# jim-berend/semanticlens

Hardware: AMD Instinct MI355X
Metric: images/sec concept-db build (higher is better)
Workload: dtype f32 (encoder GEMMs split-bf16x3, fp32 accumulate)

## Files before the change

include/semanticlens_amd.h:

```cpp
#ifndef SEMANTICLENS_AMD_H
#define SEMANTICLENS_AMD_H

#include <stddef.h>
#include <stdint.h>

#ifdef __cplusplus
extern "C" {
#endif

#define SL_ABI_VERSION 1

#define SL_E_INVALID (-1)
#define SL_E_HIP (-2)
#define SL_E_UNSUPPORTED (-3)

#define SL_F32 0
#define SL_F16 1
#define SL_BF16 2

#define SL_CONV_MAX 0
#define SL_CONV_MEAN 1
#define SL_CONV_SUM 2

#define SL_TOK_MEAN 0
// ... 181 lines not shown
int sl_condition_init(const float* d_act, int64_t B, int64_t C, int64_t S, int64_t sb, int64_t sc, int64_t ss,
                      const int64_t* d_channels, int rf, float* d_out, int64_t ob, int64_t oc, int64_t os, void* stream);

int sl_activation_heat_boxes(const float* d_act, int64_t B, int64_t C, int64_t S, int64_t sb, int64_t sc, int64_t ss,
                             int64_t prefix, int64_t gh, int64_t gw, const int64_t* d_rows, const int64_t* d_channels,
                             int64_t P, int64_t H, int64_t W, int kernel_size, float crop_th, float* d_heat, int32_t* d_box,
                             void* d_ws, size_t ws_bytes, void* stream);
int sl_heat_boxes(const float* d_heat, int64_t P, int64_t H, int64_t W, int kernel_size, float crop_th, int32_t* d_box,
                  void* d_ws, size_t ws_bytes, void* stream);

int sl_batchnorm_infer(const float* d_x, int64_t B, int64_t C, int64_t HW, const float* d_mean, const float* d_var,
                       const float* d_scale, const float* d_bias, double eps, int relu, float* d_y, void* stream);
int sl_batchnorm_infer_add_relu(const float* d_x, const float* d_residual, int64_t B, int64_t C, int64_t HW,
                                const float* d_mean, const float* d_var, const float* d_scale, const float* d_bias,
                                double eps, float* d_y, void* stream);
int sl_batchnorm_infer_add_bn_relu(const float* d_xa, const float* d_mean_a, const float* d_var_a, const float* d_scale_a,
                                   const float* d_bias_a, double eps_a, const float* d_xb, const float* d_mean_b,
                                   const float* d_var_b, const float* d_scale_b, const float* d_bias_b, double eps_b, int64_t B,
                                   int64_t C, int64_t HW, float* d_y, void* stream);
int sl_batchnorm_infer_relu_maxpool(const float* d_x, int64_t B, int64_t C, int64_t H, int64_t W, const float* d_mean,
                                    const float* d_var, const float* d_scale, const float* d_bias, double eps, int kh, int kw,
                                    int sh, int sw, int ph, int pw, float* d_y, void* stream);

int sl_topk_init(float* d_vals, int64_t* d_ids, int64_t R, int64_t k, void* stream);
int sl_topk_merge(float* d_vals, int64_t* d_ids, int64_t R, int64_t k, const float* d_cand, int64_t ld, int64_t B,
                  int64_t id_base, void* d_ws, size_t ws_bytes, void* stream);
size_t sl_topk_merge_ws_bytes(int64_t R, int64_t k, int64_t B);
int sl_topk_merge_states(float* d_vals, int64_t* d_ids, int64_t R, int64_t k, const float* d_other_vals,
                         const int64_t* d_other_ids, int64_t M, void* stream);

int sl_mutualmax_merge(uint64_t* d_row_state, uint64_t* d_col_state, int64_t R, int64_t B, const float* d_cand, int64_t ld,
                       int64_t row_id_base, int64_t col_id_base, void* stream);
int sl_mutualmax_finish(const uint64_t* d_state, int64_t n, float* d_vals, int64_t* d_ids, void* stream);

int sl_segmax_merge(uint64_t* d_state, int64_t state_ld, int64_t G, int64_t R, int64_t B, const float* d_cand, int64_t ld,
                    const int32_t* d_row_seg, int64_t row_id_base, void* stream);

int sl_unionfind_init(int32_t* d_parent, int32_t* d_degree, int32_t* d_status, int64_t n, void* stream);
int sl_threshold_union_merge(int32_t* d_parent, int32_t* d_degree, int32_t* d_status, int64_t n, const float* d_cand, int64_t ld,
                             int64_t R, int64_t B, int64_t row_id_base, int64_t col_id_base, float threshold, void* stream);
int sl_unionfind_flatten(int32_t* d_parent, int64_t n, int32_t* d_status, void* stream);
int sl_group_min_merge(uint32_t* d_state, const int32_t* d_labels, int64_t n, const float* d_cand, int64_t ld, int64_t R, int64_t B,
                       int64_t row_id_base, int64_t col_id_base, void* stream);
int sl_group_min_finish(const uint32_t* d_state, const int32_t* d_labels, int64_t n, float* d_cohesion, void* stream);

int sl_softmax_init(double* d_state, int64_t R, void* stream);
// ... 33 lines not shown
```

semanticlens_amd/_native.py:

```python
from __future__ import annotations

import ctypes
import math
import operator
import os
from collections import namedtuple
from pathlib import Path

import torch

_PKG = Path(__file__).resolve().parent
LIB_PATH = _PKG / "lib" / "libsemanticlens_hip.so"

SL_F32, SL_F16, SL_BF16 = 0, 1, 2
SL_CONV_MAX, SL_CONV_MEAN, SL_CONV_SUM = 0, 1, 2
SL_TOK_MEAN, SL_TOK_ABSMEAN, SL_TOK_MAX, SL_TOK_ABSMAX, SL_TOK_TOKEN = 0, 1, 2, 3, 4
SL_TIES_TOTAL, SL_TIES_ATEN = 0, 1
SL_MAX_SLOTS = 16
SL_PROF_REDUCE, SL_PROF_MERGE, SL_PROF_GEMM, SL_PROF_GATHER, SL_PROF_SCORES, SL_PROF_BATCHNORM, SL_PROF_TOPK = 0, 1, 2, 3, 4, 5, 6
SL_PROF_SOFTMAX = 7
SL_ACT_NONE, SL_ACT_GELU, SL_ACT_QUICKGELU, SL_ACT_GELU_TANH = 0, 1, 2, 3
TIE_MODES = {"total": SL_TIES_TOTAL, "aten": SL_TIES_ATEN}
SL_PP_PLAN_STRIDE = 16
PP_RESIZE_MODES = {"shortest": 0, "squash": 1}
# ... 72 lines not shown
    "sl_attention_pool_q": (_int, [_vp, _i64, _vp, _i64, _i64, _i64, _i64, _i64, _i64, _vp, _vp]),
    "sl_tokens_from_map": (_int, [_vp, _i64, _i64, _i64, _vp, _vp, _vp]),
    "sl_split_elems": (_sz, [_i64, _i64]),
    "sl_split_bf16": (_int, [_vp, _vp, _i64, _i64, _vp, _vp]),
    "sl_linear_bf16x3": (_int, [_vp, _i64, _i64, _vp, _i64, _vp, _int, _vp, _vp, _vp, _i64, _i64, _i64, _i64, _vp, _vp]),
    "sl_broadcast_row": (_int, [_vp, _vp, _i64, _i64, _i64, _vp, _vp]),
    "sl_embed_tokens": (_int, [_vp, _i64, _vp, _i64, _i64, _i64, _vp, _vp, _vp]),
    "sl_preprocess_plan": (_int, [_vp, _vp, _i64, _int, _int, _int, _vp, _vp]),
    "sl_preprocess": (_int, [_vp, _vp, _i64, _int, _int, _i64, _i64, _vp, _vp, _vp, _vp, _vp, _sz, _vp]),
    "sl_render_ws_bytes": (_sz, [_i64, _i64, _i64]),
    "sl_render_heatmaps": (_int, [_vp, _i64, _i64, _i64, _i64, _vp, _int, ctypes.c_float, ctypes.c_float, ctypes.c_double, _int, _int,
                                  _vp, _vp, _vp, _vp, _vp, _sz, _vp]),
    "sl_condition_init": (_int, [_vp, _i64, _i64, _i64, _i64, _i64, _i64, _vp, _int, _vp, _i64, _i64, _i64, _vp]),
    "sl_preprocess_plan_rois": (_int, [_vp, _vp, _i64, _vp, _vp, _i64, _int, _int, _int, _vp, _vp]),
    "sl_activation_heat_boxes": (_int, [_vp, _i64, _i64, _i64, _i64, _i64, _i64, _i64, _i64, _i64, _vp, _vp, _i64, _i64, _i64, _int,
                                        ctypes.c_float, _vp, _vp, _vp, _sz, _vp]),
    "sl_heat_boxes": (_int, [_vp, _i64, _i64, _i64, _int, ctypes.c_float, _vp, _vp, _sz, _vp]),
    "sl_batchnorm_infer": (_int, [_vp, _i64, _i64, _i64, _vp, _vp, _vp, _vp, ctypes.c_double, _int, _vp, _vp]),
    "sl_batchnorm_infer_add_relu": (_int, [_vp, _vp, _i64, _i64, _i64, _vp, _vp, _vp, _vp, ctypes.c_double, _vp, _vp]),
    "sl_batchnorm_infer_add_bn_relu": (_int, [_vp, _vp, _vp, _vp, _vp, ctypes.c_double, _vp, _vp, _vp, _vp, _vp, ctypes.c_double, _i64, _i64,
                                              _i64, _vp, _vp]),
    "sl_batchnorm_infer_relu_maxpool": (_int, [_vp, _i64, _i64, _i64, _i64, _vp, _vp, _vp, _vp, ctypes.c_double, _int, _int, _int,
                                               _int, _int, _int, _vp, _vp]),
    "sl_topk_init": (_int, [_vp, _vp, _i64, _i64, _vp]),
    "sl_topk_merge": (_int, [_vp, _vp, _i64, _i64, _vp, _i64, _i64, _i64, _vp, _sz, _vp]),
    "sl_topk_merge_ws_bytes": (_sz, [_i64, _i64, _i64]),
    "sl_topk_merge_states": (_int, [_vp, _vp, _i64, _i64, _vp, _vp, _i64, _vp]),
    "sl_softmax_init": (_int, [_vp, _i64, _vp]),
    "sl_softmax_merge": (_int, [_vp, _i64, _vp, _i64, _i64, ctypes.c_double, _vp, _sz, _vp]),
    "sl_softmax_merge_ws_bytes": (_sz, [_i64, _i64]),
    "sl_softmax_finish": (_int, [_vp, _i64, ctypes.c_double, _vp, _i64, _vp, _vp, _vp, _vp]),
    "sl_rank_merge": (_int, [_vp, _i64, _i64, _vp, _i64, _i64, _i64, _vp, _vp, _vp]),
    "sl_rank_merge_splits": (_i64, [_i64, _i64]),
    "sl_mutualmax_merge": (_int, [_vp, _vp, _i64, _i64, _vp, _i64, _i64, _i64, _vp]),
    "sl_mutualmax_finish": (_int, [_vp, _i64, _vp, _vp, _vp]),
    "sl_segmax_merge": (_int, [_vp, _i64, _i64, _i64, _i64, _vp, _i64, _vp, _i64, _vp]),
    "sl_unionfind_init": (_int, [_vp, _vp, _vp, _i64, _vp]),
    "sl_threshold_union_merge": (_int, [_vp, _vp, _vp, _i64, _vp, _i64, _i64, _i64, _i64, _i64, ctypes.c_float, _vp]),
    "sl_unionfind_flatten": (_int, [_vp, _i64, _vp, _vp]),
    "sl_group_min_merge": (_int, [_vp, _vp, _i64, _vp, _i64, _i64, _i64, _i64, _i64, _vp]),
    "sl_group_min_finish": (_int, [_vp, _vp, _i64, _vp, _vp]),
    "sl_cosine_nt": (_int, [_vp, _i64, _vp, _i64, _i64, _vp, _vp, _sz, _vp]),
    "sl_cosine_nt_ws_bytes": (_sz, [_i64, _i64, _i64]),
    "sl_prof_enable": (_int, [_int]),
    "sl_prof_reset": (_int, []),
    "sl_prof_read": (_int, [_int, ctypes.POINTER(ctypes.c_double), ctypes.POINTER(_i64), ctypes.POINTER(ctypes.c_double)]),
# ... 1213 lines not shown
                                                  *(_ptr(p) for p in bn_b[:4]), float(bn_b[4]), B, C, H * W, _ptr(out), _stream(xa))
    _check(rc, "sl_batchnorm_infer_add_bn_relu")
    return out


BN_POOL_MAX_WIDTH = 4096
BN_POOL_STAGE_BYTES = 64 * 1024


def bn_pool_supported(kernel_size, stride, padding) -> bool:
    return all(k in (2, 3) and s in (1, 2) and 0 <= p <= k // 2 for k, s, p in zip(kernel_size, stride, padding))


def batchnorm_infer_relu_maxpool(x: torch.Tensor, mean: torch.Tensor, var: torch.Tensor, weight: torch.Tensor, bias: torch.Tensor,
                                 eps: float, kernel_size, stride, padding) -> torch.Tensor:
    B, C, H, W = x.shape
    (kh, kw), (sh, sw), (ph, pw) = kernel_size, stride, padding
    oh, ow = ((n + 2 * p - k) // s + 1 if s > 0 else 0 for n, k, s, p in ((H, kh, sh, ph), (W, kw, sw, pw)))
    out = torch.empty((B, C, max(oh, 0), max(ow, 0)), dtype=x.dtype, device=x.device)
    with _on(x.device):
        rc = lib().sl_batchnorm_infer_relu_maxpool(_ptr(x), B, C, H, W, _ptr(mean), _ptr(var), _ptr(weight), _ptr(bias),
                                                   float(eps), kh, kw, sh, sw, ph, pw, _ptr(out), _stream(x))
    _check(rc, "sl_batchnorm_infer_relu_maxpool")
    return out


def prof_enable(on: bool = True):
    _check(lib().sl_prof_enable(1 if on else 0), "sl_prof_enable")


def prof_reset():
    _check(lib().sl_prof_reset(), "sl_prof_reset")


def prof_read(family: int):
    ms, n, w = ctypes.c_double(), _i64(), ctypes.c_double()
    _check(lib().sl_prof_read(family, ctypes.byref(ms), ctypes.byref(n), ctypes.byref(w)), "sl_prof_read")
    return ms.value, n.value, w.value


POLY2_MAX_N = 128


POLYK_MAX_N = 1024
POLYK_MAX_CLUSTERS = 16
POLYK_MAX_COMPONENTS = 65535
# ... 504 lines not shown
```

semanticlens_amd/component_visualization/_bn_fuse.py:

```python
from __future__ import annotations

import inspect
import operator
import os
import warnings
import weakref

import torch
import torch.nn as nn
import torch.nn.functional as F

from .. import _native as N

_BN_FORWARD = nn.modules.batchnorm._BatchNorm.forward
_PLANS: "weakref.WeakKeyDictionary[nn.Module, _Plan]" = weakref.WeakKeyDictionary()
_ADDS = (operator.add, operator.iadd, torch.add)
_RELUS = (F.relu, torch.relu, torch.relu_)
_POOL_ARGS = ("kernel_size", "stride", "padding", "dilation", "ceil_mode", "return_indices")


def enabled() -> bool:
    return os.environ.get("SEMANTICLENS_AMD_FUSE_BN", "1") != "0"


def _plain_bn(m) -> bool:
    return isinstance(m, nn.BatchNorm2d) and type(m).forward is _BN_FORWARD


def _plain_relu(m) -> bool:
    return isinstance(m, nn.ReLU) and type(m).forward is nn.ReLU.forward


def _plain_seq(m) -> bool:
    return isinstance(m, nn.Sequential) and type(m).forward is nn.Sequential.forward


def _plain_pool(m) -> bool:
    return isinstance(m, nn.MaxPool2d) and type(m).forward is nn.MaxPool2d.forward


def _pair(v):
    if isinstance(v, int) and not isinstance(v, bool):
        return (v, v)
    if isinstance(v, (tuple, list)) and len(v) == 2 and all(isinstance(e, int) and not isinstance(e, bool) for e in v):
        return tuple(v)
    return None


def _pool_params(kernel_size, stride=None, padding=0, dilation=1, ceil_mode=False, return_indices=False):
    if ceil_mode or return_indices or _pair(dilation) != (1, 1):
        return None
    k, p = _pair(kernel_size), _pair(padding)
    s = k if stride is None or stride == [] or stride == () else _pair(stride)
    if k is None or s is None or p is None or not N.bn_pool_supported(k, s, p):
        return None
    return k, s, p


def _hooked(m: nn.Module) -> bool:
    mod = nn.modules.module
    return bool(m._forward_hooks or m._forward_pre_hooks or mod._global_forward_hooks or mod._global_forward_pre_hooks)


def _streamable(t) -> bool:
    return (isinstance(t, torch.Tensor) and t.is_cuda and t.dtype is torch.float32 and t.dim() == 4 and not t.requires_grad
            and t.is_contiguous() and not t.is_contiguous(memory_format=torch.channels_last) and t.data_ptr() % 16 == 0)


class _Site:

    __slots__ = ("bn", "verified", "dropped", "no_pool")

    def __init__(self, bn: nn.BatchNorm2d):
        self.bn = bn
        self.verified: set = set()
        self.dropped = False
        self.no_pool = False

    def eligible(self, x) -> bool:
        bn = self.bn
        if self.dropped or bn.training or torch.is_grad_enabled() or not enabled():
            return False
        if not _streamable(x) or not 0 < x.numel() <= N.BN_MAX_ELEMENTS or x.shape[1] > N.BN_MAX_CHANNELS:
            return False
        if not torch.backends.cudnn.enabled or torch.is_autocast_enabled():
            return False
        for p in (bn.running_mean, bn.running_var, bn.weight, bn.bias):
            if p is None or p.dtype is not torch.float32 or p.device != x.device or not p.is_contiguous() or p.numel() != x.shape[1]:
                return False
        return True

    def run(self, x, relu: bool, other=None, bn_first: bool = True):
        bn = self.bn
        out = N.batchnorm_infer(x, bn.running_mean, bn.running_var, bn.weight, bn.bias, bn.eps, relu=relu, residual=other)
        key = (relu, other is not None, (x.shape[2] * x.shape[3]) % 4 == 0)
        if key in self.verified:
            return out
        ref = F.batch_norm(x, bn.running_mean, bn.running_var, bn.weight, bn.bias, False, 0.0, bn.eps)
        if other is not None:
            ref = ref + other if bn_first else other + ref
        if relu:
            ref = torch.relu_(ref)
        if torch.equal(out.view(torch.int32), ref.view(torch.int32)):
            self.verified.add(key)
            return out
        self.dropped = True
        warnings.warn(
            f"the fused BatchNorm kernel did not reproduce PyTorch's result bit for bit on a {tuple(x.shape)} input "
            f"(relu={relu}, residual={other is not None}); this BatchNorm2d runs unfused from now on.", RuntimeWarning, stacklevel=3)
        return ref

# ... 71 lines not shown
    def forward(self, x, xb):
        a, b = self.single.site, self.shortcut
        if (self.ready() and a.eligible(x) and b.eligible(xb) and xb.shape == x.shape and xb.device == x.device
                and x.shape[1] <= N.BN_DUAL_MAX_CHANNELS):
            return self.run(x, xb)
        return self.single(x, b.bn(xb))

    def run(self, x, xb):
        bn_first = self.single.bn_first
        left, right = ((x, self.single.site.bn), (xb, self.shortcut.bn)) if bn_first else ((xb, self.shortcut.bn), (x, self.single.site.bn))
        out = N.batchnorm_infer_add_bn_relu(left[0], _bn_args(left[1]), right[0], _bn_args(right[1]))
        key = ((x.shape[2] * x.shape[3]) % 4 == 0, bn_first)
        if key in self.verified:
            return out
        ref = torch.relu_(F.batch_norm(left[0], *_bn_args(left[1])[:4], False, 0.0, left[1].eps)
                          + F.batch_norm(right[0], *_bn_args(right[1])[:4], False, 0.0, right[1].eps))
        if torch.equal(out.view(torch.int32), ref.view(torch.int32)):
            self.verified.add(key)
            return out
        self.dropped = True
        warnings.warn(
            f"the fused BatchNorm + BatchNorm + add + ReLU kernel did not reproduce PyTorch's result bit for bit on {tuple(x.shape)} "
            f"inputs; this shortcut's BatchNorm2d runs on its own from now on.", RuntimeWarning, stacklevel=3)
        return ref


class _FusedPool(nn.Module):

    def __init__(self, inner: _Fused, pool):
        super().__init__()
        self.__dict__.update(inner=inner, pool=pool)

    def forward(self, x):
        inner, pool = self.inner, self.pool
        site, relu = inner.site, inner.relu
        if isinstance(pool, nn.Module):
            params = _pool_params(*(getattr(pool, name) for name in _POOL_ARGS))
            hooked = _hooked(pool)
        else:
            params, hooked = _pool_params(**pool), False
        if (params is not None and not hooked and not _hooked(site.bn) and not (isinstance(relu, nn.Module) and _hooked(relu))
                and site.eligible(x) and site.pool_eligible(x, params)):
            return site.run_pool(x, params)
        out = inner(x)
        return pool(out) if isinstance(pool, nn.Module) else F.max_pool2d(out, **pool)


def _trace(parent: nn.Module, sites: dict, dual: bool = False):
    from torch import fx

    class InplaceProxy(fx.Proxy):
        pass

    for name in ("iadd", "isub", "imul", "itruediv"):
        op = getattr(operator, name)
        setattr(InplaceProxy, f"__{name}__",
                lambda self, other, op=op: self.tracer.create_proxy("call_function", op, (self, other), {}))

    class LeafTracer(fx.Tracer):
        def is_leaf_module(self, m, qualname):
            return True

        def proxy(self, node):
            return InplaceProxy(node, self)

    params = list(inspect.signature(parent.forward).parameters.values())
    if any(p.kind is not p.POSITIONAL_OR_KEYWORD or p.default is not p.empty for p in params):
        return None
    graph = LeafTracer().trace(parent)
    gm = fx.GraphModule(parent, graph)
    mods = dict(parent.named_modules())
# ... 9 lines not shown

    def pool_of(node, source):
        if not node.args or node.args[0] is not source:
            return None
        if node.op == "call_module" and _plain_pool(mods.get(node.target)) and len(node.args) == 1 and not node.kwargs:
            return mods[node.target]
        if node.op == "call_function" and node.target is F.max_pool2d and len(node.args) <= 1 + len(_POOL_ARGS):
            given = dict(zip(_POOL_ARGS, node.args[1:]))
            if set(given) & set(node.kwargs) or not set(node.kwargs) <= set(_POOL_ARGS):
                return None
            given.update(node.kwargs)
            flat = [e for v in given.values() for e in (v if isinstance(v, (tuple, list)) else (v,))]
            if "kernel_size" in given and not any(isinstance(e, fx.Node) for e in flat):
                return given
        return None

    def shortcut_of(node, add):
        seq = mods.get(node.target) if node.op == "call_module" else None
        if not _plain_seq(seq) or node.kwargs or len(node.args) != 1 or set(node.users) != {add}:
            return None
        children = list(seq.children())
        return sites.get(children[-1]) if len(children) >= 2 else None

    n_fused, duals = 0, []
    for node in list(graph.nodes):
        if node.op != "call_module" or mods.get(node.target) not in sites or node.kwargs or len(node.args) != 1:
            continue
        if len(node.users) != 1:
            continue
        site, user = sites[mods[node.target]], next(iter(node.users))
        last, fused, args, stale = user, None, None, None
        if relu_of(user) is not None:
            fused, args = _Fused(site, relu_of(user)), (node.args[0],)
            follower = next(iter(user.users)) if len(user.users) == 1 else None
            pool = pool_of(follower, user) if follower is not None else None
            if pool is not None:
                last, fused = follower, _FusedPool(fused, pool)
        elif (user.op == "call_function" and user.target in _ADDS and not user.kwargs and len(user.args) == 2
              and all(isinstance(a, fx.Node) for a in user.args) and user.args[0] is not user.args[1] and len(user.users) == 1):
            last = next(iter(user.users))
            if relu_of(last) is None:
                continue
            bn_first = user.args[0] is node
            if user.target is operator.iadd and not bn_first:
                continue
            fused = _Fused(site, relu_of(last), user.target, bn_first)
            other = user.args[1] if bn_first else user.args[0]
            args = (node.args[0], other)
            shortcut = shortcut_of(other, user) if dual else None
            if shortcut is not None:
                seq, tail = mods[other.target], other.args[0]
                with graph.inserting_before(other):
                    for child_name in list(seq._modules)[:-1]:
                        tail = graph.call_module(f"{other.target}.{child_name}", (tail,))
                fused, args, stale = _FusedDual(fused, shortcut, seq), (node.args[0], tail), other
                duals.append(fused)
        if fused is None:
            continue
        name = f"_sl_fused_{n_fused}"
        n_fused += 1
        gm.add_submodule(name, fused)
        with graph.inserting_before(last):
            new = graph.call_module(name, args)
        last.replace_all_uses_with(new)
        graph.erase_node(last)
        if last is not user:
            graph.erase_node(user)
        graph.erase_node(node)
        if stale is not None:
            graph.erase_node(stale)
    if not n_fused or (dual and not duals):
        return None
    graph.lint()
    gm.recompile()
    return (gm, duals) if dual else gm


def _owner_forward(parent: nn.Module, gm, training: bool, dual=None):
    own = type(parent).forward

    def forward(*args, **kwargs):
        if parent.training is training:
            if dual is not None and all(f.ready() for f in dual[1]):
                return dual[0].forward(*args, **kwargs)
            return gm.forward(*args, **kwargs)
        return own(parent, *args, **kwargs)

    return forward


class _Plan:
    def __init__(self, model: nn.Module):
        self.module_ids = tuple(id(m) for m in model.modules())
        self.sites = {m: _Site(m) for m in model.modules() if _plain_bn(m) and m is not model}
        self.parents: list = []
        self.duals: dict = {}
        for parent in model.modules():
            if "forward" in parent.__dict__ or not any(child in self.sites for child in parent.children()):
                continue
            try:
                gm = _trace(parent, self.sites)
            except Exception:
                gm = None
            if gm is None:
                continue
            self.parents.append((weakref.ref(parent), gm, parent.training))
            if any(_plain_seq(c) and len(c) >= 2 and c[-1] in self.sites for c in parent.children()):
                try:
                    dual = _trace(parent, self.sites, dual=True)
                except Exception:
                    dual = None
                if dual is not None:
                    self.duals[len(self.parents) - 1] = dual

    def valid_for(self, model: nn.Module) -> bool:
        return self.module_ids == tuple(id(m) for m in model.modules())


def substitute(model: nn.Module):
    if not enabled() or not isinstance(model, nn.Module):
        return None
    plan = _PLANS.get(model)
    if plan is None or not plan.valid_for(model):
        plan = _PLANS[model] = _Plan(model)
    swapped = []
    for bn, site in plan.sites.items():
        if "forward" not in bn.__dict__:
            bn.forward = _bn_forward(site)
            swapped.append(bn)
    for i, (ref, gm, training) in enumerate(plan.parents):
        parent = ref()
        if parent is not None and "forward" not in parent.__dict__:
            parent.forward = _owner_forward(parent, gm, training, plan.duals.get(i))
            swapped.append(parent)

    def undo():
        for m in swapped:
            m.__dict__.pop("forward", None)
        swapped.clear()

    return undo
```

semanticlens_amd/csrc/batchnorm.hip:

```cpp
#include "common.hpp"

namespace sl {
namespace {

typedef float f4 __attribute__((ext_vector_type(4)));

enum { EPI_PLAIN = 0, EPI_RELU = 1, EPI_ADD_RELU = 2, EPI_ADD_BN_RELU = 3 };
enum { POL_PLAIN = 0, POL_NT_STORE = 1, POL_NT_BOTH = 2 };

constexpr int kBlock = 256;
constexpr int kUnroll = 4;
constexpr int64_t kMaxC = 4096;
constexpr int64_t kMaxCDual = 2048;
constexpr int64_t kLdsPerCu = 160 * 1024;
constexpr size_t kDualResidentFrom = 32 * 1024;
constexpr int64_t kMaxTotal = (int64_t)1 << 31;

__device__ inline float bn_inv_std(float var, double eps) { return __builtin_amdgcn_rsqf(fabsf(var + (float)eps)); }

__device__ inline float bn_value(float x, const f4 k) {
  const float xhat = (x - k.x) * k.y;
  return __fmaf_rn(k.z, xhat, k.w);
}

__device__ inline float relu_clamp(float v) { return v != v ? v : fmaxf(v, 0.f); }

__device__ inline float add_as_aten(float a, float b) {
  float r;
  asm("v_add_f32_e32 %0, %1, %2" : "=v"(r) : "v"(b), "v"(a));
  return r;
}

struct BnParams {
  const float *mean, *var, *scale, *bias;
  double eps;
};

template <int EPI>
__device__ inline float bn_finish(float x, const f4 k, float r, const f4 kb) {
  float y = bn_value(x, k);
  if constexpr (EPI == EPI_ADD_RELU) y = y + r;
  if constexpr (EPI == EPI_ADD_BN_RELU) y = add_as_aten(y, bn_value(r, kb));
  if constexpr (EPI != EPI_PLAIN) y = relu_clamp(y);
  return y;
}

template <int POL>
__device__ inline f4 ld4(const f4* p) {
  if constexpr (POL == POL_NT_BOTH) return __builtin_nontemporal_load(p);
  return *p;
}
template <int POL>
__device__ inline void st4(f4* p, f4 v) {
  if constexpr (POL != POL_PLAIN)
    __builtin_nontemporal_store(v, p);
  else
    *p = v;
}
template <int POL>
__device__ inline float ld1(const float* p) {
  if constexpr (POL == POL_NT_BOTH) return __builtin_nontemporal_load(p);
  return *p;
}
template <int POL>
__device__ inline void st1(float* p, float v) {
  if constexpr (POL != POL_PLAIN)
    __builtin_nontemporal_store(v, p);
  else
    *p = v;
}

template <int EPI, bool ALIGNED, int POL>
__global__ __launch_bounds__(kBlock) void batchnorm_kernel(const float* __restrict__ x, const float* __restrict__ res,
                                                           float* __restrict__ y, const BnParams a, const BnParams b, uint32_t C,
                                                           uint32_t HW, uint32_t total) {
  constexpr bool HAS_RES = EPI == EPI_ADD_RELU || EPI == EPI_ADD_BN_RELU;
  constexpr bool DUAL = EPI == EPI_ADD_BN_RELU;
  extern __shared__ f4 tab[];
  for (uint32_t c = threadIdx.x; c < C; c += kBlock) {
    tab[c] = f4{a.mean[c], bn_inv_std(a.var[c], a.eps), a.scale[c], a.bias[c]};
    if constexpr (DUAL) tab[C + c] = f4{b.mean[c], bn_inv_std(b.var[c], b.eps), b.scale[c], b.bias[c]};
  }
  __syncthreads();
  const uint32_t second = DUAL ? C : 0u;

  const uint32_t lane = threadIdx.x & 63;
  const uint32_t wave = blockIdx.x * (kBlock / 64) + (uint32_t)__builtin_amdgcn_readfirstlane((int)(threadIdx.x >> 6));
  const uint32_t nwaves = gridDim.x * (kBlock / 64);
  const uint32_t n4 = total / 4;
  const uint32_t per_plane = ALIGNED ? HW / 4 : 1;
  const f4* x4 = reinterpret_cast<const f4*>(x);
  const f4* r4 = reinterpret_cast<const f4*>(res);
  f4* y4 = reinterpret_cast<f4*>(y);

  for (uint32_t base = wave * (64 * kUnroll); base < n4; base += nwaves * (64 * kUnroll)) {
    f4 v[kUnroll], r[kUnroll];
#pragma unroll
    for (int u = 0; u < kUnroll; ++u) {
      const uint32_t i = base + u * 64 + lane;
      if (i < n4) {
        v[u] = ld4<POL>(x4 + i);
        if constexpr (HAS_RES) r[u] = ld4<POL>(r4 + i);
      }
    }
// ... 358 lines not shown
```

Measured before the change: 7563.

## Fuse 1x1 64->256 conv with BatchNorm, residual add and ReLU in bottleneck tails

Adds HIP kernels that compute the 64->256 1x1 convolution at ResNet bottleneck tails and apply BatchNorm, the residual add and ReLU in the same pass. A dual variant also folds in the downsample shortcut's 1x1 conv and its BatchNorm. The FX trace pass is extended to rewrite these conv+BN+add+ReLU patterns. The aim is to avoid writing and re-reading the conv output and to skip separate library GEMM launches. Each new input shape is checked bit-for-bit against PyTorch's own result, and the module falls back to the unfused path if they differ.

```diff
diff --git a/include/semanticlens_amd.h b/include/semanticlens_amd.h
--- a/include/semanticlens_amd.h
+++ b/include/semanticlens_amd.h
@@ -227,6 +227,16 @@
                                     const float* d_var, const float* d_scale, const float* d_bias, double eps, int kh, int kw,
                                     int sh, int sw, int ph, int pw, float* d_y, void* stream);
 
+int sl_conv1x1_64_256(const float* d_x, const float* d_w, int64_t N, int64_t HW, int split, const int32_t* d_korder, float* d_y,
+                      void* stream);
+int sl_conv1x1_bn_add_relu(const float* d_x, const float* d_w, const float* d_mean, const float* d_var, const float* d_scale,
+                           const float* d_bias, double eps, const float* d_identity, int64_t N, int64_t HW, float* d_y,
+                           void* stream);
+int sl_conv1x1_bn_add_conv1x1_bn_relu(const float* d_xa, const float* d_wa, const float* d_mean_a, const float* d_var_a,
+                                      const float* d_scale_a, const float* d_bias_a, double eps_a, const float* d_xb,
+                                      const float* d_wb, const float* d_mean_b, const float* d_var_b, const float* d_scale_b,
+                                      const float* d_bias_b, double eps_b, int64_t N, int64_t HW, float* d_y, void* stream);
+
 int sl_topk_init(float* d_vals, int64_t* d_ids, int64_t R, int64_t k, void* stream);
 int sl_topk_merge(float* d_vals, int64_t* d_ids, int64_t R, int64_t k, const float* d_cand, int64_t ld, int64_t B,
                   int64_t id_base, void* d_ws, size_t ws_bytes, void* stream);
diff --git a/semanticlens_amd/_native.py b/semanticlens_amd/_native.py
--- a/semanticlens_amd/_native.py
+++ b/semanticlens_amd/_native.py
@@ -118,6 +118,10 @@
                                               _i64, _vp, _vp]),
     "sl_batchnorm_infer_relu_maxpool": (_int, [_vp, _i64, _i64, _i64, _i64, _vp, _vp, _vp, _vp, ctypes.c_double, _int, _int, _int,
                                                _int, _int, _int, _vp, _vp]),
+    "sl_conv1x1_64_256": (_int, [_vp, _vp, _i64, _i64, _int, _vp, _vp, _vp]),
+    "sl_conv1x1_bn_add_relu": (_int, [_vp, _vp, _vp, _vp, _vp, _vp, ctypes.c_double, _vp, _i64, _i64, _vp, _vp]),
+    "sl_conv1x1_bn_add_conv1x1_bn_relu": (_int, [_vp, _vp, _vp, _vp, _vp, _vp, ctypes.c_double, _vp, _vp, _vp, _vp, _vp, _vp,
+                                                 ctypes.c_double, _i64, _i64, _vp, _vp]),
     "sl_topk_init": (_int, [_vp, _vp, _i64, _i64, _vp]),
     "sl_topk_merge": (_int, [_vp, _vp, _i64, _i64, _vp, _i64, _i64, _i64, _vp, _sz, _vp]),
     "sl_topk_merge_ws_bytes": (_sz, [_i64, _i64, _i64]),
@@ -1377,6 +1381,78 @@
         rc = lib().sl_batchnorm_infer_relu_maxpool(_ptr(x), B, C, H, W, _ptr(mean), _ptr(var), _ptr(weight), _ptr(bias),
                                                    float(eps), kh, kw, sh, sw, ph, pw, _ptr(out), _stream(x))
     _check(rc, "sl_batchnorm_infer_relu_maxpool")
+    return out
+
+
+CONV_TAIL_IN, CONV_TAIL_OUT = 64, 256
+CONV_TAIL_SPLITS = 7
+CONV_TAIL_MAX_ELEMENTS = (1 << 31) - 1
+
+
+def _conv_tail_operands(what: str, x: torch.Tensor, w: torch.Tensor):
+    if x.dim() != 4 or x.shape[1] != CONV_TAIL_IN or w.numel() != CONV_TAIL_IN * CONV_TAIL_OUT or w.shape[:2] != (CONV_TAIL_OUT,
+                                                                                                                 CONV_TAIL_IN):
+        raise ValueError(f"{what}: a (N, {CONV_TAIL_IN}, H, W) input and a ({CONV_TAIL_OUT}, {CONV_TAIL_IN}[, 1, 1]) weight expected, "
+                         f"got {tuple(x.shape)} and {tuple(w.shape)}")
+    for t in (x, w):
+        if t.dtype is not torch.float32 or not t.is_cuda or t.device != x.device or not t.is_contiguous() or t.data_ptr() % 16:
+            raise ValueError(f"{what}: operands must be contiguous fp32 on one HIP device, 16-byte aligned")
+    B, _, H, W = x.shape
+    return B, H, W
+
+
+def _conv_tail_out(x: torch.Tensor) -> torch.Tensor:
+    return torch.empty((x.shape[0], CONV_TAIL_OUT, x.shape[2], x.shape[3]), dtype=x.dtype, device=x.device)
+
+
+def _conv_tail_bn(what: str, x: torch.Tensor, bn):
+    for p in bn[:4]:
+        if p.dtype is not torch.float32 or p.device != x.device or not p.is_contiguous() or p.numel() != CONV_TAIL_OUT:
+            raise ValueError(f"{what}: per-channel tensors must be contiguous fp32 of {CONV_TAIL_OUT} elements on {x.device}")
+
+
+def conv1x1_64_256(x: torch.Tensor, w: torch.Tensor, split: int, k_order: torch.Tensor | None = None) -> torch.Tensor:
+    B, H, W = _conv_tail_operands("conv1x1_64_256", x, w)
+    out = _conv_tail_out(x)
+    if k_order is not None and (k_order.dtype is not torch.int32 or k_order.device != x.device or k_order.numel() != CONV_TAIL_IN
+                                or not k_order.is_contiguous()
+                                or sorted(k_order.tolist()) != list(range(CONV_TAIL_IN))):
+        raise ValueError("conv1x1_64_256: k_order must be a permutation of 0..63 as contiguous int32 on the input's device")
+    with _on(x.device):
+        rc = lib().sl_conv1x1_64_256(_ptr(x), _ptr(w), B, H * W, int(split), _ptr(k_order), _ptr(out), _stream(x))
+    _check(rc, "sl_conv1x1_64_256")
+    return out
+
+
+def conv1x1_bn_add_relu(x: torch.Tensor, w: torch.Tensor, bn, identity: torch.Tensor) -> torch.Tensor:
+    B, H, W = _conv_tail_operands("conv1x1_bn_add_relu", x, w)
+    out = _conv_tail_out(x)
+    _conv_tail_bn("conv1x1_bn_add_relu", x, bn)
+    if (identity.shape != out.shape or identity.dtype is not torch.float32 or identity.device != x.device
+            or not identity.is_contiguous() or identity.data_ptr() % 16):
+        raise ValueError(f"conv1x1_bn_add_relu: the identity must be contiguous fp32 of shape {tuple(out.shape)} on {x.device}")
+    with _on(x.device):
+        rc = lib().sl_conv1x1_bn_add_relu(_ptr(x), _ptr(w), *(_ptr(p) for p in bn[:4]), float(bn[4]), _ptr(identity), B, H * W,
+                                          _ptr(out), _stream(x))
+    _check(rc, "sl_conv1x1_bn_add_relu")
+    return out
+
+
+def conv1x1_bn_add_conv1x1_bn_relu(xa: torch.Tensor, wa: torch.Tensor, bn_a, xb: torch.Tensor, wb: torch.Tensor,
+                                   bn_b) -> torch.Tensor:
+    what = "conv1x1_bn_add_conv1x1_bn_relu"
+    B, H, W = _conv_tail_operands(what, xa, wa)
+    _conv_tail_operands(what, xb, wb)
+    if xb.shape != xa.shape or xb.device != xa.device:
+        raise ValueError(f"{what}: two inputs of one shape and device expected, got {tuple(xa.shape)} and {tuple(xb.shape)}")
+    _conv_tail_bn(what, xa, bn_a)
+    _conv_tail_bn(what, xa, bn_b)
+    out = _conv_tail_out(xa)
+    with _on(xa.device):
+        rc = lib().sl_conv1x1_bn_add_conv1x1_bn_relu(_ptr(xa), _ptr(wa), *(_ptr(p) for p in bn_a[:4]), float(bn_a[4]), _ptr(xb),
+                                                     _ptr(wb), *(_ptr(p) for p in bn_b[:4]), float(bn_b[4]), B, H * W,
+                                                     _ptr(out), _stream(xa))
+    _check(rc, what)
     return out
 
 
diff --git a/semanticlens_amd/component_visualization/_bn_fuse.py b/semanticlens_amd/component_visualization/_bn_fuse.py
--- a/semanticlens_amd/component_visualization/_bn_fuse.py
+++ b/semanticlens_amd/component_visualization/_bn_fuse.py
@@ -23,6 +23,10 @@
     return os.environ.get("SEMANTICLENS_AMD_FUSE_BN", "1") != "0"
 
 
+def conv_enabled() -> bool:
+    return enabled() and os.environ.get("SEMANTICLENS_AMD_FUSE_CONV", "1") != "0"
+
+
 def _plain_bn(m) -> bool:
     return isinstance(m, nn.BatchNorm2d) and type(m).forward is _BN_FORWARD
 
@@ -37,6 +41,13 @@
 
 def _plain_pool(m) -> bool:
     return isinstance(m, nn.MaxPool2d) and type(m).forward is nn.MaxPool2d.forward
+
+
+def _tail_conv(m) -> bool:
+    return (isinstance(m, nn.Conv2d) and type(m).forward is nn.Conv2d.forward and m.in_channels == N.CONV_TAIL_IN
+            and m.out_channels == N.CONV_TAIL_OUT and tuple(m.kernel_size) == (1, 1) and tuple(m.stride) == (1, 1)
+            and m.padding in ((0, 0), 0) and tuple(m.dilation) == (1, 1) and m.groups == 1 and m.bias is None
+            and m.padding_mode == "zeros")
 
 
 def _pair(v):
@@ -67,6 +78,18 @@
             and t.is_contiguous() and not t.is_contiguous(memory_format=torch.channels_last) and t.data_ptr() % 16 == 0)
 
 
+def _conv_operands(conv: nn.Conv2d, x) -> bool:
+    w = conv.weight
+    return (_streamable(x) and x.shape[1] == N.CONV_TAIL_IN and x.numel() > 0
+            and x.numel() // N.CONV_TAIL_IN * N.CONV_TAIL_OUT <= N.CONV_TAIL_MAX_ELEMENTS and isinstance(w, torch.Tensor)
+            and w.dtype is torch.float32 and w.device == x.device and w.is_contiguous() and w.data_ptr() % 16 == 0
+            and tuple(w.shape) == (N.CONV_TAIL_OUT, N.CONV_TAIL_IN, 1, 1))
+
+
+def _solver_key(x):
+    return tuple(x.shape), torch.backends.cudnn.benchmark, torch.backends.cudnn.deterministic
+
+
 class _Site:
 
     __slots__ = ("bn", "verified", "dropped", "no_pool")
@@ -78,15 +101,18 @@
         self.no_pool = False
 
     def eligible(self, x) -> bool:
+        if not _streamable(x) or not 0 < x.numel() <= N.BN_MAX_ELEMENTS or x.shape[1] > N.BN_MAX_CHANNELS:
+            return False
+        return self.usable(x.device, x.shape[1])
+
+    def usable(self, device, channels: int) -> bool:
         bn = self.bn
         if self.dropped or bn.training or torch.is_grad_enabled() or not enabled():
-            return False
-        if not _streamable(x) or not 0 < x.numel() <= N.BN_MAX_ELEMENTS or x.shape[1] > N.BN_MAX_CHANNELS:
             return False
         if not torch.backends.cudnn.enabled or torch.is_autocast_enabled():
             return False
         for p in (bn.running_mean, bn.running_var, bn.weight, bn.bias):
-            if p is None or p.dtype is not torch.float32 or p.device != x.device or not p.is_contiguous() or p.numel() != x.shape[1]:
+            if p is None or p.dtype is not torch.float32 or p.device != device or not p.is_contiguous() or p.numel() != channels:
                 return False
         return True
 
@@ -204,6 +230,85 @@
         warnings.warn(
             f"the fused BatchNorm + BatchNorm + add + ReLU kernel did not reproduce PyTorch's result bit for bit on {tuple(x.shape)} "
             f"inputs; this shortcut's BatchNorm2d runs on its own from now on.", RuntimeWarning, stacklevel=3)
+        return ref
+
+
+def _unhooked_tail(single: _Fused) -> bool:
+    relu = single.relu
+    return not _hooked(single.site.bn) and not (isinstance(relu, nn.Module) and _hooked(relu))
+
+
+class _FusedConv(nn.Module):
+
+    def __init__(self, single: _Fused, conv: nn.Conv2d):
+        super().__init__()
+        self.__dict__.update(single=single, conv=conv, verified=set(), dropped=False)
+
+    def ready(self) -> bool:
+        return (conv_enabled() and not self.dropped and _tail_conv(self.conv) and not _hooked(self.conv)
+                and _unhooked_tail(self.single))
+
+    def forward(self, x, other):
+        site = self.single.site
+        if (self.ready() and _conv_operands(self.conv, x) and site.usable(x.device, N.CONV_TAIL_OUT) and _streamable(other)
+                and other.device == x.device
+                and tuple(other.shape) == (x.shape[0], N.CONV_TAIL_OUT, x.shape[2], x.shape[3])):
+            return self.run(x, other)
+        return self.single(self.conv(x), other)
+
+    def run(self, x, other):
+        bn, w, bn_first = self.single.site.bn, self.conv.weight, self.single.bn_first
+        out = N.conv1x1_bn_add_relu(x, w, _bn_args(bn), other)
+        key = (_solver_key(x), bn_first)
+        if key in self.verified:
+            return out
+        ref = F.batch_norm(F.conv2d(x, w), *_bn_args(bn)[:4], False, 0.0, bn.eps)
+        ref = torch.relu_(ref + other if bn_first else other + ref)
+        if torch.equal(out.view(torch.int32), ref.view(torch.int32)):
+            self.verified.add(key)
+            return out
+        self.dropped = True
+        warnings.warn(
+            f"the fused convolution + BatchNorm + add + ReLU kernel did not reproduce PyTorch's result bit for bit on a "
+            f"{tuple(x.shape)} input; this convolution runs on its own from now on.", RuntimeWarning, stacklevel=3)
+        return ref
+
+
+class _FusedConvDual(nn.Module):
+
+    def __init__(self, dual: _FusedDual, conv: nn.Conv2d, shortcut_conv: nn.Conv2d):
+        super().__init__()
+        self.__dict__.update(dual=dual, conv=conv, shortcut_conv=shortcut_conv, verified=set(), dropped=False)
+
+    def ready(self) -> bool:
+        return (conv_enabled() and not self.dropped and self.dual.ready() and len(self.dual.children_seen) == 2
+                and self.dual.children_seen[0] is self.shortcut_conv and _tail_conv(self.conv) and _tail_conv(self.shortcut_conv)
+                and not _hooked(self.conv) and not _hooked(self.shortcut_conv))
+
+    def forward(self, x, xb):
+        a, b = self.dual.single.site, self.dual.shortcut
+        if (self.ready() and _conv_operands(self.conv, x) and _conv_operands(self.shortcut_conv, xb) and xb.shape == x.shape
+                and xb.device == x.device and a.usable(x.device, N.CONV_TAIL_OUT) and b.usable(x.device, N.CONV_TAIL_OUT)):
+            return self.run(x, xb)
+        return self.dual(self.conv(x), self.shortcut_conv(xb))
+
+    def run(self, x, xb):
+        single, bn_first = self.dual.single, self.dual.single.bn_first
+        ours, theirs = (x, self.conv.weight, single.site.bn), (xb, self.shortcut_conv.weight, self.dual.shortcut.bn)
+        left, right = (ours, theirs) if bn_first else (theirs, ours)
+        out = N.conv1x1_bn_add_conv1x1_bn_relu(left[0], left[1], _bn_args(left[2]), right[0], right[1], _bn_args(right[2]))
+        key = (_solver_key(x), bn_first)
+        if key in self.verified:
+            return out
+        ref = torch.relu_(F.batch_norm(F.conv2d(left[0], left[1]), *_bn_args(left[2])[:4], False, 0.0, left[2].eps)
+                          + F.batch_norm(F.conv2d(right[0], right[1]), *_bn_args(right[2])[:4], False, 0.0, right[2].eps))
+        if torch.equal(out.view(torch.int32), ref.view(torch.int32)):
+            self.verified.add(key)
+            return out
+        self.dropped = True
+        warnings.warn(
+            f"the fused kernel of two convolutions, their BatchNorms, add and ReLU did not reproduce PyTorch's result bit for bit "
+            f"on {tuple(x.shape)} inputs; these convolutions run on their own from now on.", RuntimeWarning, stacklevel=3)
         return ref
 
 
@@ -228,7 +333,7 @@
         return pool(out) if isinstance(pool, nn.Module) else F.max_pool2d(out, **pool)
 
 
-def _trace(parent: nn.Module, sites: dict, dual: bool = False):
+def _trace(parent: nn.Module, sites: dict, dual: bool = False, conv: bool = False):
     from torch import fx
 
     class InplaceProxy(fx.Proxy):
@@ -284,14 +389,20 @@
         children = list(seq.children())
         return sites.get(children[-1]) if len(children) >= 2 else None
 
-    n_fused, duals = 0, []
+    def conv_of(node, consumer):
+        m = mods.get(node.target) if isinstance(node, fx.Node) and node.op == "call_module" else None
+        if not _tail_conv(m) or node.kwargs or len(node.args) != 1 or set(node.users) != {consumer}:
+            return None
+        return m
+
+    n_fused, duals, convs = 0, [], []
     for node in list(graph.nodes):
         if node.op != "call_module" or mods.get(node.target) not in sites or node.kwargs or len(node.args) != 1:
             continue
         if len(node.users) != 1:
             continue
         site, user = sites[mods[node.target]], next(iter(node.users))
-        last, fused, args, stale = user, None, None, None
+        last, fused, args, stale = user, None, None, []
         if relu_of(user) is not None:
             fused, args = _Fused(site, relu_of(user)), (node.args[0],)
             follower = next(iter(user.users)) if len(user.users) == 1 else None
@@ -315,8 +426,18 @@
                 with graph.inserting_before(other):
                     for child_name in list(seq._modules)[:-1]:
                         tail = graph.call_module(f"{other.target}.{child_name}", (tail,))
-                fused, args, stale = _FusedDual(fused, shortcut, seq), (node.args[0], tail), other
+                fused, args, stale = _FusedDual(fused, shortcut, seq), (node.args[0], tail), [other]
                 duals.append(fused)
+            ours = conv_of(node.args[0], node) if conv else None
+            if ours is not None and isinstance(fused, _Fused):
+                fused, args, stale = _FusedConv(fused, ours), (node.args[0].args[0], other), [node.args[0]]
+                convs.append(fused)
+            elif ours is not None and isinstance(fused, _FusedDual) and len(fused.children_seen) == 2 and _tail_conv(
+                    fused.children_seen[0]):
+                duals.remove(fused)
+                stale += [node.args[0], args[1]]
+                fused, args = _FusedConvDual(fused, ours, fused.children_seen[0]), (node.args[0].args[0], other.args[0])
+                convs.append(fused)
         if fused is None:
             continue
         name = f"_sl_fused_{n_fused}"
@@ -329,20 +450,24 @@
         if last is not user:
             graph.erase_node(user)
         graph.erase_node(node)
-        if stale is not None:
-            graph.erase_node(stale)
-    if not n_fused or (dual and not duals):
+        for dead in stale:
+            graph.erase_node(dead)
+    if not n_fused or (conv and not convs) or (dual and not conv and not duals):
         return None
     graph.lint()
     gm.recompile()
+    if conv:
+        return gm, convs + duals
     return (gm, duals) if dual else gm
 
 
-def _owner_forward(parent: nn.Module, gm, training: bool, dual=None):
+def _owner_forward(parent: nn.Module, gm, training: bool, dual=None, conv=None):
     own = type(parent).forward
 
     def forward(*args, **kwargs):
         if parent.training is training:
+            if conv is not None and all(f.ready() for f in conv[1]):
+                return conv[0].forward(*args, **kwargs)
             if dual is not None and all(f.ready() for f in dual[1]):
                 return dual[0].forward(*args, **kwargs)
             return gm.forward(*args, **kwargs)
@@ -357,6 +482,7 @@
         self.sites = {m: _Site(m) for m in model.modules() if _plain_bn(m) and m is not model}
         self.parents: list = []
         self.duals: dict = {}
+        self.convs: dict = {}
         for parent in model.modules():
             if "forward" in parent.__dict__ or not any(child in self.sites for child in parent.children()):
                 continue
@@ -374,6 +500,13 @@
                     dual = None
                 if dual is not None:
                     self.duals[len(self.parents) - 1] = dual
+            if any(_tail_conv(c) for c in parent.children()):
+                try:
+                    conv = _trace(parent, self.sites, dual=len(self.parents) - 1 in self.duals, conv=True)
+                except Exception:
+                    conv = None
+                if conv is not None:
+                    self.convs[len(self.parents) - 1] = conv
 
     def valid_for(self, model: nn.Module) -> bool:
         return self.module_ids == tuple(id(m) for m in model.modules())
@@ -393,7 +526,7 @@
     for i, (ref, gm, training) in enumerate(plan.parents):
         parent = ref()
         if parent is not None and "forward" not in parent.__dict__:
-            parent.forward = _owner_forward(parent, gm, training, plan.duals.get(i))
+            parent.forward = _owner_forward(parent, gm, training, plan.duals.get(i), plan.convs.get(i))
             swapped.append(parent)
 
     def undo():
diff --git a/semanticlens_amd/csrc/batchnorm.hip b/semanticlens_amd/csrc/batchnorm.hip
--- a/semanticlens_amd/csrc/batchnorm.hip
+++ b/semanticlens_amd/csrc/batchnorm.hip
@@ -1,11 +1,8 @@
-#include "common.hpp"
+#include "bn_apply.hpp"
 
 namespace sl {
 namespace {
 
-typedef float f4 __attribute__((ext_vector_type(4)));
-
-enum { EPI_PLAIN = 0, EPI_RELU = 1, EPI_ADD_RELU = 2, EPI_ADD_BN_RELU = 3 };
 enum { POL_PLAIN = 0, POL_NT_STORE = 1, POL_NT_BOTH = 2 };
 
 constexpr int kBlock = 256;
@@ -16,34 +13,6 @@
 constexpr size_t kDualResidentFrom = 32 * 1024;
 constexpr int64_t kMaxTotal = (int64_t)1 << 31;
 
-__device__ inline float bn_inv_std(float var, double eps) { return __builtin_amdgcn_rsqf(fabsf(var + (float)eps)); }
-
-__device__ inline float bn_value(float x, const f4 k) {
-  const float xhat = (x - k.x) * k.y;
-  return __fmaf_rn(k.z, xhat, k.w);
-}
-
-__device__ inline float relu_clamp(float v) { return v != v ? v : fmaxf(v, 0.f); }
-
-__device__ inline float add_as_aten(float a, float b) {
-  float r;
-  asm("v_add_f32_e32 %0, %1, %2" : "=v"(r) : "v"(b), "v"(a));
-  return r;
-}
-
-struct BnParams {
-  const float *mean, *var, *scale, *bias;
-  double eps;
-};
-
-template <int EPI>
-__device__ inline float bn_finish(float x, const f4 k, float r, const f4 kb) {
-  float y = bn_value(x, k);
-  if constexpr (EPI == EPI_ADD_RELU) y = y + r;
-  if constexpr (EPI == EPI_ADD_BN_RELU) y = add_as_aten(y, bn_value(r, kb));
-  if constexpr (EPI != EPI_PLAIN) y = relu_clamp(y);
-  return y;
-}
 
 template <int POL>
 __device__ inline f4 ld4(const f4* p) {
@@ -78,8 +47,8 @@
   constexpr bool DUAL = EPI == EPI_ADD_BN_RELU;
   extern __shared__ f4 tab[];
   for (uint32_t c = threadIdx.x; c < C; c += kBlock) {
-    tab[c] = f4{a.mean[c], bn_inv_std(a.var[c], a.eps), a.scale[c], a.bias[c]};
-    if constexpr (DUAL) tab[C + c] = f4{b.mean[c], bn_inv_std(b.var[c], b.eps), b.scale[c], b.bias[c]};
+    tab[c] = bn_constants(a, c);
+    if constexpr (DUAL) tab[C + c] = bn_constants(b, c);
   }
   __syncthreads();
   const uint32_t second = DUAL ? C : 0u;
diff --git a/semanticlens_amd/csrc/bn_apply.hpp b/semanticlens_amd/csrc/bn_apply.hpp
--- /dev/null
+++ b/semanticlens_amd/csrc/bn_apply.hpp
@@ -0,0 +1,41 @@
+#pragma once
+#include "common.hpp"
+
+namespace sl {
+
+enum { EPI_PLAIN = 0, EPI_RELU = 1, EPI_ADD_RELU = 2, EPI_ADD_BN_RELU = 3 };
+
+__device__ inline float bn_inv_std(float var, double eps) { return __builtin_amdgcn_rsqf(fabsf(var + (float)eps)); }
+
+__device__ inline float bn_value(float x, const f4 k) {
+  const float xhat = (x - k.x) * k.y;
+  return __fmaf_rn(k.z, xhat, k.w);
+}
+
+__device__ inline float relu_clamp(float v) { return v != v ? v : fmaxf(v, 0.f); }
+
+__device__ inline float add_as_aten(float a, float b) {
+  float r;
+  asm("v_add_f32_e32 %0, %1, %2" : "=v"(r) : "v"(b), "v"(a));
+  return r;
+}
+
+struct BnParams {
+  const float *mean, *var, *scale, *bias;
+  double eps;
+};
+
+__device__ inline f4 bn_constants(const BnParams& p, uint32_t c) {
+  return f4{p.mean[c], bn_inv_std(p.var[c], p.eps), p.scale[c], p.bias[c]};
+}
+
+template <int EPI>
+__device__ inline float bn_finish(float x, const f4 k, float r, const f4 kb) {
+  float y = bn_value(x, k);
+  if constexpr (EPI == EPI_ADD_RELU) y = y + r;
+  if constexpr (EPI == EPI_ADD_BN_RELU) y = add_as_aten(y, bn_value(r, kb));
+  if constexpr (EPI != EPI_PLAIN) y = relu_clamp(y);
+  return y;
+}
+
+}
diff --git a/semanticlens_amd/csrc/conv_tail.hip b/semanticlens_amd/csrc/conv_tail.hip
--- /dev/null
+++ b/semanticlens_amd/csrc/conv_tail.hip
@@ -0,0 +1,284 @@
+#include "bn_apply.hpp"
+
+namespace sl {
+namespace {
+
+enum { FORM_CONV = 0, FORM_ADD_RELU = 1, FORM_DUAL = 2 };
+
+constexpr int kCi = 64, kCo = 256;
+constexpr int kSteps = kCi / 4;
+constexpr int kNt = kCo / 16;
+constexpr int kBlock = 512, kWaves = kBlock / 64;
+constexpr int kTilePx = 32;
+constexpr int kWFloats = kCi * kCo;
+constexpr int kSplits = 7;
+constexpr int64_t kMaxTotal = (int64_t)1 << 31;
+
+template <int S, bool INTER>
+__device__ constexpr int chain_of(int s) {
+  return INTER ? s % S : s / (kSteps / S);
+}
+
+template <int S, bool PAIR>
+__device__ inline f4 combine(const f4 (&p)[S]) {
+  if constexpr (S == 1)
+    return p[0];
+  else if constexpr (S == 2)
+    return p[0] + p[1];
+  else if constexpr (PAIR)
+    return (p[0] + p[1]) + (p[2] + p[3]);
+  else
+    return ((p[0] + p[1]) + p[2]) + p[3];
+}
+
+__device__ inline void stage_w(float* wl, const float* __restrict__ w, const int32_t* __restrict__ order) {
+  for (int d = threadIdx.x; d < kWFloats; d += kBlock) {
+    const int sj = d & 3, lane = (d >> 2) & 63, s4 = (d >> 8) & 3, nt = d >> 10;
+    const int slot = 4 * (4 * s4 + sj) + (lane >> 4);
+    const int k = order ? order[slot] : slot;
+    wl[d] = w[(16 * nt + (lane & 15)) * kCi + k];
+  }
+}
+
+__device__ inline void load_a(float (&a)[2][kSteps], const float* __restrict__ xn, const uint32_t (&koff)[kSteps], uint32_t p0,
+                              uint32_t HW, uint32_t j) {
+#pragma unroll
+  for (int t = 0; t < 2; ++t) {
+    const uint32_t px = p0 + 16 * t + j, at = px < HW ? px : HW - 1;
+#pragma unroll
+    for (int s = 0; s < kSteps; ++s) a[t][s] = xn[koff[s] + at];
+  }
+}
+
+template <int S, bool INTER, bool PAIR>
+__device__ inline void product(const float (&a)[2][kSteps], const f4* wl4, f4 (&r)[2]) {
+  f4 p[2][S];
+#pragma unroll
+  for (int t = 0; t < 2; ++t)
+#pragma unroll
+    for (int c = 0; c < S; ++c) p[t][c] = f4{0.f, 0.f, 0.f, 0.f};
+#pragma unroll
+  for (int s4 = 0; s4 < kSteps / 4; ++s4) {
+    const f4 b = wl4[s4 * 64];
+#pragma unroll
+    for (int sj = 0; sj < 4; ++sj) {
+      const int s = 4 * s4 + sj, c = chain_of<S, INTER>(s);
+#pragma unroll
+      for (int t = 0; t < 2; ++t) p[t][c] = __builtin_amdgcn_mfma_f32_16x16x4f32(a[t][s], b[sj], p[t][c], 0, 0, 0);
+    }
+  }
+#pragma unroll
+  for (int t = 0; t < 2; ++t) r[t] = combine<S, PAIR>(p[t]);
+}
+
+template <bool ALIGNED>
+__device__ inline f4 load_px4(const float* __restrict__ plane, uint32_t px, uint32_t HW) {
+  f4 v = {0.f, 0.f, 0.f, 0.f};
+  if constexpr (ALIGNED) {
+    v = __builtin_nontemporal_load(reinterpret_cast<const f4*>(plane + (px < HW ? px : HW - 4)));
+  } else {
+#pragma unroll
+    for (int e = 0; e < 4; ++e)
+      if (px + e < HW) v[e] = __builtin_nontemporal_load(plane + px + e);
+  }
+  return v;
+}
+template <bool ALIGNED>
+__device__ inline void store_px4(float* __restrict__ plane, uint32_t px, uint32_t HW, f4 v) {
+  if constexpr (ALIGNED) {
+    if (px < HW) *reinterpret_cast<f4*>(plane + px) = v;
+  } else {
+#pragma unroll
+    for (int e = 0; e < 4; ++e)
+      if (px + e < HW) plane[px + e] = v[e];
+  }
+}
+
+template <int FORM, int S, bool INTER, bool PAIR, bool ALIGNED>
+__global__ __launch_bounds__(kBlock) void conv_tail_kernel(const float* __restrict__ xa, const float* __restrict__ wa,
+                                                           const BnParams bna, const float* __restrict__ other,
+                                                           const float* __restrict__ wb, const BnParams bnb,
+                                                           float* __restrict__ y, const int32_t* __restrict__ order, uint32_t N,
+                                                           uint32_t HW, uint32_t tiles) {
+  constexpr bool DUAL = FORM == FORM_DUAL;
+  constexpr int EPI = DUAL ? EPI_ADD_BN_RELU : EPI_ADD_RELU;
+  extern __shared__ f4 lds[];
+  float* wl = reinterpret_cast<float*>(lds);
+  f4* tab = lds + (DUAL ? 2 : 1) * (kWFloats / 4);
+  stage_w(wl, wa, order);
+  if constexpr (DUAL) stage_w(wl + kWFloats, wb, order);
+  if constexpr (FORM != FORM_CONV) {
+    for (uint32_t c = threadIdx.x; c < (uint32_t)kCo; c += kBlock) {
+      tab[c] = bn_constants(bna, c);
+      if constexpr (DUAL) tab[kCo + c] = bn_constants(bnb, c);
+    }
+  }
+  __syncthreads();
+
+  const uint32_t lane = threadIdx.x & 63, g = lane >> 4, j = lane & 15;
+  const uint32_t wave = blockIdx.x * kWaves + (uint32_t)__builtin_amdgcn_readfirstlane((int)(threadIdx.x >> 6));
+  const uint32_t nwaves = gridDim.x * kWaves, nwork = N * tiles;
+  uint32_t koff[kSteps];
+#pragma unroll
+  for (int s = 0; s < kSteps; ++s) koff[s] = (uint32_t)(order ? order[4 * s + g] : 4 * s + (int)g) * HW;
+  const f4* wl4 = lds + lane;
+
+  for (uint32_t work = wave; work < nwork; work += nwaves) {
+    const uint32_t n = work / tiles, p0 = (work - n * tiles) * kTilePx;
+    float a[2][kSteps], ab[DUAL ? 2 : 1][kSteps];
+    load_a(a, xa + (size_t)n * kCi * HW, koff, p0, HW, j);
+    if constexpr (DUAL) load_a(ab, other + (size_t)n * kCi * HW, koff, p0, HW, j);
+    const size_t row0 = ((size_t)n * kCo + j) * HW;
+    f4 ahead[2];
+    if constexpr (FORM == FORM_ADD_RELU) {
+#pragma unroll
+      for (int t = 0; t < 2; ++t) ahead[t] = load_px4<ALIGNED>(other + row0, p0 + 16 * t + 4 * g, HW);
+    }
+#pragma unroll
+    for (int nt = 0; nt < kNt; ++nt) {
+      const uint32_t co = 16 * nt + j;
+      const size_t row = row0 + (size_t)(16 * nt) * HW;
+      f4 r[2], rb[2];
+      if constexpr (FORM == FORM_ADD_RELU) {
+#pragma unroll
+        for (int t = 0; t < 2; ++t) rb[t] = ahead[t];
+        if (nt + 1 < kNt) {
+#pragma unroll
+          for (int t = 0; t < 2; ++t) ahead[t] = load_px4<ALIGNED>(other + row + (size_t)16 * HW, p0 + 16 * t + 4 * g, HW);
+        }
+        __builtin_amdgcn_sched_barrier(0);
+      }
+      if constexpr (FORM == FORM_CONV) __builtin_amdgcn_sched_barrier(0);
+      product<S, INTER, PAIR>(a, wl4 + nt * 256, r);
+      if constexpr (DUAL) product<S, INTER, PAIR>(ab, wl4 + kWFloats / 4 + nt * 256, rb);
+      f4 k = {}, kb = {};
+      if constexpr (FORM != FORM_CONV) k = tab[co];
+      if constexpr (DUAL) kb = tab[kCo + co];
+#pragma unroll
+      for (int t = 0; t < 2; ++t) {
+        f4 o = r[t];
+        if constexpr (FORM != FORM_CONV) {
+#pragma unroll
+          for (int e = 0; e < 4; ++e) o[e] = bn_finish<EPI>(r[t][e], k, rb[t][e], kb);
+        }
+        store_px4<ALIGNED>(y + row, p0 + 16 * t + 4 * g, HW, o);
+      }
+    }
+  }
+}
+
+struct NoProf {
+  hipEvent_t start = nullptr, stop = nullptr;
+};
+
+template <int FORM, int S, bool INTER, bool PAIR, bool ALIGNED, class Prof>
+int launch_instance(Prof& prof, dim3 grid, size_t lds, hipStream_t st, const float* xa, const float* wa, const BnParams& bna,
+                    const float* other, const float* wb, const BnParams& bnb, float* y, const int32_t* order, uint32_t N,
+                    uint32_t HW, uint32_t tiles) {
+  SL_CHECK_HIP(hipFuncSetAttribute(reinterpret_cast<const void*>(&conv_tail_kernel<FORM, S, INTER, PAIR, ALIGNED>),
+                                   hipFuncAttributeMaxDynamicSharedMemorySize, (int)lds));
+  SL_LAUNCH(prof, (conv_tail_kernel<FORM, S, INTER, PAIR, ALIGNED>), grid, dim3(kBlock), lds, st, xa, wa, bna, other, wb, bnb, y,
+            order, N, HW, tiles);
+  return 0;
+}
+
+template <int FORM, bool ALIGNED, class Prof>
+int launch_split(int split, Prof& prof, dim3 grid, size_t lds, hipStream_t st, const float* xa, const float* wa,
+                 const BnParams& bna, const float* other, const float* wb, const BnParams& bnb, float* y, const int32_t* order,
+                 uint32_t N, uint32_t HW, uint32_t tiles) {
+#define SL_CT(S_, I_, P_) \
+  return launch_instance<FORM, S_, I_, P_, ALIGNED>(prof, grid, lds, st, xa, wa, bna, other, wb, bnb, y, order, N, HW, tiles)
+  if constexpr (FORM != FORM_CONV) {
+    SL_CT(1, false, false);
+  } else {
+    switch (split) {
+      case 0: SL_CT(1, false, false);
+      case 1: SL_CT(2, false, false);
+      case 2: SL_CT(2, true, false);
+      case 3: SL_CT(4, false, false);
+      case 4: SL_CT(4, false, true);
+      case 5: SL_CT(4, true, false);
+      default: SL_CT(4, true, true);
+    }
+  }
+#undef SL_CT
+}
+
+int blocks_per_cu(int form) { return form == FORM_DUAL ? 1 : 2; }
+
+int launch_conv_tail(int form, int split, const float* xa, const float* wa, const BnParams& bna, const float* other,
+                     const float* wb, const BnParams& bnb, float* y, const int32_t* order, int64_t N, int64_t HW, hipStream_t st,
+                     const char* who) {
+  SL_REQUIRE(N >= 0 && HW >= 0, "%s: negative shape", who);
+  SL_REQUIRE(split >= 0 && split < kSplits, "%s: split %d is not one of 0..%d", who, split, kSplits - 1);
+  const int64_t total = N * kCo * HW;
+  if (total == 0) return 0;
+  SL_REQUIRE(total < kMaxTotal, "%s: %lld output elements exceed the supported maximum of 2^31 - 1", who, (long long)total);
+  SL_REQUIRE(xa && wa && y && (form == FORM_CONV || other), "%s: null pointer", who);
+  SL_REQUIRE(form == FORM_CONV || (bna.mean && bna.var && bna.scale && bna.bias), "%s: null pointer", who);
+  SL_REQUIRE(form != FORM_DUAL || (wb && bnb.mean && bnb.var && bnb.scale && bnb.bias), "%s: null pointer", who);
+  SL_REQUIRE((((uintptr_t)xa | (uintptr_t)y | (uintptr_t)other | (uintptr_t)wa | (uintptr_t)wb) & 15) == 0,
+             "%s: tensors must be 16-byte aligned", who);
+  const int64_t tiles = (HW + kTilePx - 1) / kTilePx, nwork = N * tiles;
+  int64_t blocks = (nwork + kWaves - 1) / kWaves;
+  const int64_t cap = (int64_t)num_cus() * blocks_per_cu(form);
+  if (blocks > cap) blocks = cap;
+  const dim3 grid((unsigned)blocks);
+  const size_t lds = (size_t)(form == FORM_DUAL ? 2 : 1) * (kWFloats * 4 + (form == FORM_CONV ? 0 : kCo * sizeof(f4)));
+  const uint32_t n = (uint32_t)N, hw = (uint32_t)HW, nt = (uint32_t)tiles;
+  int rc;
+  if (form == FORM_CONV) {
+    NoProf none;
+    rc = HW % 4 == 0 ? launch_split<FORM_CONV, true>(split, none, grid, lds, st, xa, wa, bna, other, wb, bnb, y, order, n, hw, nt)
+                     : launch_split<FORM_CONV, false>(split, none, grid, lds, st, xa, wa, bna, other, wb, bnb, y, order, n, hw, nt);
+  } else {
+    const double bytes = ((double)total + (double)N * kCi * HW * (form == FORM_DUAL ? 2 : 1) + (form == FORM_ADD_RELU ? (double)total : 0.0)) * 4;
+    ProfScope prof(SL_PROF_BATCHNORM, st, bytes);
+#define SL_CT_FORM(F_)                                                                                                           \
+  rc = HW % 4 == 0 ? launch_split<F_, true>(split, prof, grid, lds, st, xa, wa, bna, other, wb, bnb, y, order, n, hw, nt)        \
+                   : launch_split<F_, false>(split, prof, grid, lds, st, xa, wa, bna, other, wb, bnb, y, order, n, hw, nt)
+    if (form == FORM_ADD_RELU)
+      SL_CT_FORM(FORM_ADD_RELU);
+    else
+      SL_CT_FORM(FORM_DUAL);
+#undef SL_CT_FORM
+  }
+  if (rc) return rc;
+  SL_CHECK_HIP(hipGetLastError());
+  if (form == FORM_DUAL) {
+    ProfScope second(SL_PROF_BATCHNORM, st, 0.0);
+    if (second.start) {
+      SL_CHECK_HIP(hipEventRecord(second.start, st));
+      SL_CHECK_HIP(hipEventRecord(second.stop, st));
+    }
+  }
+  return 0;
+}
+
+}
+}
+
+using namespace sl;
+
+SL_API int sl_conv1x1_64_256(const float* d_x, const float* d_w, int64_t N, int64_t HW, int split, const int32_t* d_korder,
+                             float* d_y, void* stream) {
+  return launch_conv_tail(FORM_CONV, split, d_x, d_w, BnParams{}, nullptr, nullptr, BnParams{}, d_y, d_korder, N, HW,
+                          (hipStream_t)stream, "sl_conv1x1_64_256");
+}
+
+SL_API int sl_conv1x1_bn_add_relu(const float* d_x, const float* d_w, const float* d_mean, const float* d_var,
+                                  const float* d_scale, const float* d_bias, double eps, const float* d_identity, int64_t N,
+                                  int64_t HW, float* d_y, void* stream) {
+  return launch_conv_tail(FORM_ADD_RELU, 0, d_x, d_w, BnParams{d_mean, d_var, d_scale, d_bias, eps}, d_identity, nullptr,
+                          BnParams{}, d_y, nullptr, N, HW, (hipStream_t)stream, "sl_conv1x1_bn_add_relu");
+}
+
+SL_API int sl_conv1x1_bn_add_conv1x1_bn_relu(const float* d_xa, const float* d_wa, const float* d_mean_a, const float* d_var_a,
+                                             const float* d_scale_a, const float* d_bias_a, double eps_a, const float* d_xb,
+                                             const float* d_wb, const float* d_mean_b, const float* d_var_b,
+                                             const float* d_scale_b, const float* d_bias_b, double eps_b, int64_t N, int64_t HW,
+                                             float* d_y, void* stream) {
+  return launch_conv_tail(FORM_DUAL, 0, d_xa, d_wa, BnParams{d_mean_a, d_var_a, d_scale_a, d_bias_a, eps_a}, d_xb, d_wb,
+                          BnParams{d_mean_b, d_var_b, d_scale_b, d_bias_b, eps_b}, d_y, nullptr, N, HW, (hipStream_t)stream,
+                          "sl_conv1x1_bn_add_conv1x1_bn_relu");
+}
```

Result: faster. 7849, median of 6 (+3.8%).
